# OpenDriveLab/kai0

Hardware: AMD Instinct MI355X
Metric: train samples/sec pi0.5 full FT (higher is better)
Workload: dtype bf16; 1 GPU; pi0.5 full fine-tune bf16, batch 32 per MI355X, 3-cam 224x224 (BASELINE.json configs[1]); global_batch=32, seq_len=1018, parallelism=dp1

## Files before the change

### include/kai0hip.h

```cpp
#ifndef KAI0HIP_H
#define KAI0HIP_H

#include <stdint.h>

#ifdef __cplusplus
extern "C" {
#endif

typedef void* kai0_stream_t;

const char* kai0_last_error(void);
int kai0_abi_version(void);
int kai0_device_info(int device, int* n_cu, int* lds_bytes, char* arch_name64);

typedef struct kai0_gemm_desc {
    const void* A;
    const void* B;
    void* C;
    int32_t M, N, K;
    int32_t a_kc, b_kc;
    int64_t lda, ldb, ldc;
    int32_t batch, batch_inner;
    int64_t sA1, sA2, sB1, sB2, sC1, sC2;
    int32_t a_rpb, b_rpb, c_rpb, _pad0;
// ... 126 lines not shown
int kai0_adarms_bwd(const void* dy, const void* dgate, const void* x, const float* mod, const float* rstd,
                    void* dx, float* dmod, const void* dres, int64_t rows, int rows_per_batch, int D,
                    kai0_stream_t stream);
int kai0_adarms_combine(const float* partials, int splits, int64_t split_stride, const void* gate_prev,
                        const void* residual, void* x_out, const float* mod, void* y, void* gate_out, int64_t rows,
                        int rows_per_batch, int D, float eps, kai0_stream_t stream);
int kai0_layernorm_fwd(const void* x, const void* w, const void* b, void* y, float* mean, float* rstd,
                       int64_t rows, int D, float eps, kai0_stream_t stream);
int kai0_layernorm_bwd(const void* dy, const void* x, const void* w, const float* mean, const float* rstd,
                       void* dx, float* dwb_partial, int dwb_blocks, const void* dres, int64_t rows, int D,
                       kai0_stream_t stream);
int kai0_reduce_partials(const float* partial, int blocks, int ncols, int64_t ld, void* out, int out_f32,
                         kai0_stream_t stream);
typedef struct kai0_reduce_item {
    const float* partial;
    void* out;
    int64_t ld;
    int32_t blocks, ncols;
    int32_t out_f32, _pad;
} kai0_reduce_item;
int kai0_reduce_partials_batch(const kai0_reduce_item* items, int n, kai0_stream_t stream);
int kai0_colsum_partials_bf16(const void* dy, int64_t M, int N, int64_t ld, float* scratch, int scratch_blocks,
                              int* blocks_used, kai0_stream_t stream);
int kai0_colsum_bf16(const void* dy, int64_t M, int N, int64_t ld, float* scratch, int scratch_blocks,
                     void* out, int out_f32, kai0_stream_t stream);

int kai0_rope_inplace(void* x, const int32_t* pos, const float* inv_freq, int B, int S, int64_t s_ld_rows,
                      int64_t row0, int H, int HD, int inverse, kai0_stream_t stream);
int kai0_rope_inplace2(void* x, int H, void* x2, int H2, const int32_t* pos, const float* inv_freq, int B, int S,
                       int64_t s_ld_rows, int64_t row0, int HD, kai0_stream_t stream);
int kai0_rope_copy(const void* src, void* dst, const int32_t* pos, const float* inv_freq, int B, int S, int H, int HD,
                   int64_t src_bs, int64_t src_ld, int64_t dst_bs, int64_t dst_ld, int64_t pos_bs, int inverse,
                   kai0_stream_t stream);

int kai0_softmax_mask_fwd(const void* scores, void* probs, const int32_t* qcode, const int32_t* kcode,
                          int B, int Sq, int H, int Sk, int64_t ld, int64_t batch_stride, int q0,
                          int64_t qcode_ld, int64_t kcode_ld, kai0_stream_t stream);
int kai0_siglip_attn_bwd(const void* q, const void* k, const void* v, const void* dO, const void* O, const void* P,
                         void* dq, void* dk, void* dv, int n_img, int S, int NH, int HD, int64_t ldp, int64_t ld_grad,
                         float scale, kai0_stream_t stream);
int kai0_siglip_attn_fwd(const void* q, const void* k, const void* v, void* o, float* lse, int n_img, int S, int NH, int HD,
                         int64_t ldq, int64_t ldk, int64_t ldv, int64_t ldo, int64_t sq, int64_t sk, int64_t sv, int64_t so,
                         float scale, kai0_stream_t stream);
int kai0_siglip_attn_bwd2(const void* q, const void* k, const void* v, const void* dO, const void* O, const float* lse,
                          void* dq, void* dk, void* dv, int n_img, int S, int NH, int HD, int64_t ld_grad, float scale,
                          kai0_stream_t stream);
int kai0_rowdot_bf16(const void* a, const void* b, float* out, int64_t rows, int D, kai0_stream_t stream);
int kai0_softmax_bwd(const void* probs, const void* dprobs, int dprobs_f32, void* dscores, int64_t rows, int Sk,
                     int64_t ld, float scale, kai0_stream_t stream);

typedef struct kai0_attn_desc {
    const void* Q; const void* K; const void* V; void* O; void* P;
    const int32_t* qcode; const int32_t* kcode;
    int32_t rows, Sk, HD, H, q0, batch, batch_inner, _pad0;
    int64_t ldq, ldk, ldv, ldo, ldp;
    int64_t sQ1, sQ2, sK1, sK2, sV1, sV2, sO1, sO2, sP;
    int64_t qcode_ld, kcode_ld;
    float scale;
    int32_t online;
    float* lse;
    int64_t s_lse;
} kai0_attn_desc;
int kai0_attn_fwd(const kai0_attn_desc* d, kai0_stream_t stream);
int kai0_attn_combine(const void* o_parts, const float* lse_parts, void* O, int parts, int rows, int HD, int64_t ldo,
                      int64_t part_stride, int64_t lse_stride, kai0_stream_t stream);
int kai0_attn_desc_size(void);

int kai0_geglu_fwd(const void* g, const void* u, void* h, int64_t n, kai0_stream_t stream);
int kai0_geglu_bwd(const void* dh, const void* g, const void* u, void* dg, void* du, int64_t n,
                   kai0_stream_t stream);
int kai0_gelu_bwd(const void* dy, const void* pre, void* dx, int64_t n, kai0_stream_t stream);
int kai0_silu_fwd_f32(const float* x, float* y, int64_t n, kai0_stream_t stream);
int kai0_silu_bwd_f32(const float* dy, const float* x, float* dx, int64_t n, kai0_stream_t stream);
int kai0_gated_fwd(const void* x, const void* y, const void* gate, void* out, int64_t rows, int rows_per_batch,
                   int D, kai0_stream_t stream);
int kai0_gated_bwd(const void* dout, const void* y, const void* gate, void* dy, void* dgate, int64_t rows,
                   int rows_per_batch, int D, kai0_stream_t stream);
int kai0_embed_gather(const void* table, const int64_t* tokens, void* out, int B, int T, int D, float scale,
                      int64_t out_bs, int64_t out_row0, int64_t out_ld, kai0_stream_t stream);
int kai0_embed_grad(const void* dout, const int64_t* tokens, void* dtable, int B, int T, int D, float scale,
                    int64_t dout_bs, int64_t dout_row0, int64_t dout_ld, kai0_stream_t stream);
int kai0_cast_f32_to_bf16(const float* x, void* y, int64_t n, kai0_stream_t stream);
int kai0_cast_bf16_to_f32(const void* x, float* y, int64_t n, kai0_stream_t stream);
int kai0_add_bf16(const void* a, const void* b, void* out, int64_t n, kai0_stream_t stream);
int kai0_add_f32(const float* a, const float* b, float* out, int64_t n, kai0_stream_t stream);
int kai0_transpose_bf16(const void* src, void* dst, int R, int C, kai0_stream_t stream);
typedef struct kai0_ck_item {
    const void* ptr;
    int64_t nbytes;
} kai0_ck_item;
int kai0_sampled_checksum(const kai0_ck_item* items_dev, int n, int stride, unsigned long long* out_dev, kai0_stream_t stream);
typedef struct kai0_pack_part {
    const void* src;
    void* dst;
    int64_t src_bs, src_ld, dst_bs, dst_ld;
    int32_t B, rows, cols, mode;
    int32_t pos_off, _pad;
} kai0_pack_part;
int kai0_pack_rows(const kai0_pack_part* parts, int n, const int32_t* pos, int64_t pos_bs, const float* inv_freq, int HD,
                   kai0_stream_t stream);
int kai0_copy_rows_bf16(const void* src, void* dst, int B, int rows, int D, int64_t src_bs, int64_t src_row0,
                        int64_t src_ld, int64_t dst_bs, int64_t dst_row0, int64_t dst_ld,
                        kai0_stream_t stream);
int kai0_patch_im2col(const float* img, float* cols, int n_img, int C, int HW, int P, kai0_stream_t stream);
int kai0_add_pos_cast(const float* x, const float* pos, void* out, int64_t rows, int n_pos, int D,
                      kai0_stream_t stream);

// ... 27 lines not shown
```

### kai0_amd/_lib.py

```python

from __future__ import annotations

import ctypes as C
import os
import pathlib

_HERE = pathlib.Path(__file__).resolve().parent
LIB_PATH = _HERE / "lib" / "libkai0hip.so"

c_p = C.c_void_p
c_i = C.c_int
c_i64 = C.c_int64
c_f = C.c_float


class GemmSeg(C.Structure):
    _fields_ = [("dst", c_p), ("ld", c_i64), ("n_begin", C.c_int32), ("_pad", C.c_int32)]


class GemmDesc(C.Structure):

    _fields_ = [
        ("A", c_p), ("B", c_p), ("C", c_p),
        ("M", C.c_int32), ("N", C.c_int32), ("K", C.c_int32),
        ("a_kc", C.c_int32), ("b_kc", C.c_int32),
        ("lda", c_i64), ("ldb", c_i64), ("ldc", c_i64),
        ("batch", C.c_int32), ("batch_inner", C.c_int32),
        ("sA1", c_i64), ("sA2", c_i64), ("sB1", c_i64), ("sB2", c_i64), ("sC1", c_i64), ("sC2", c_i64),
        ("a_rpb", C.c_int32), ("b_rpb", C.c_int32), ("c_rpb", C.c_int32), ("_pad0", C.c_int32),
        ("a_bs", c_i64), ("a_off", c_i64), ("b_bs", c_i64), ("b_off", c_i64), ("c_bs", c_i64), ("c_off", c_i64),
        ("bias", c_p), ("bias_f32", C.c_int32), ("scale", c_f),
        ("act", C.c_int32), ("out_f32", C.c_int32),
        ("pre_out", c_p), ("gate", c_p), ("gate_rpb", C.c_int32), ("accumulate", C.c_int32),
        ("gate_ld", c_i64), ("residual", c_p), ("ldr", c_i64), ("sR1", c_i64), ("sR2", c_i64),
        ("split_k", C.c_int32), ("c_nontemporal", C.c_int32), ("workspace", c_p), ("workspace_bytes", c_i64),
        ("aux1", c_p), ("aux2", c_p),
        ("nseg", C.c_int32), ("_pad2", C.c_int32), ("seg", GemmSeg * 3),
        ("rowvec", c_p), ("rv_s1", c_i64), ("rv_s2", c_i64), ("rv_ld", c_i64),
        ("B2", c_p), ("pre_out2", c_p),
        ("norm_out", c_p), ("norm_w", c_p), ("norm_b", c_p), ("norm_eps", C.c_float), ("norm_kind", C.c_int32),
        ("rope_cos", c_p), ("rope_sin", c_p), ("rope_half", C.c_int32), ("rope_n_end", C.c_int32),
        ("tile_cfg", C.c_int32), ("persist", C.c_int32), ("general_epilogue", C.c_int32), ("small_w8", C.c_int32),
    ]


class AttnDesc(C.Structure):

    _fields_ = [
        ("Q", c_p), ("K", c_p), ("V", c_p), ("O", c_p), ("P", c_p), ("qcode", c_p), ("kcode", c_p),
        ("rows", C.c_int32), ("Sk", C.c_int32), ("HD", C.c_int32), ("H", C.c_int32), ("q0", C.c_int32),
        ("batch", C.c_int32), ("batch_inner", C.c_int32), ("_pad0", C.c_int32),
        ("ldq", c_i64), ("ldk", c_i64), ("ldv", c_i64), ("ldo", c_i64), ("ldp", c_i64),
        ("sQ1", c_i64), ("sQ2", c_i64), ("sK1", c_i64), ("sK2", c_i64), ("sV1", c_i64), ("sV2", c_i64),
        ("sO1", c_i64), ("sO2", c_i64), ("sP", c_i64), ("qcode_ld", c_i64), ("kcode_ld", c_i64),
        ("scale", c_f), ("online", C.c_int32), ("lse", c_p), ("s_lse", c_i64),
    ]


class AttnBwdDesc(C.Structure):

    _fields_ = [
        ("dO", c_p), ("O", c_p), ("Q", c_p), ("K", c_p), ("V", c_p), ("lse", c_p), ("qcode", c_p), ("kcode", c_p),
        ("P", c_p), ("dS", c_p), ("dQ", c_p),
        ("batch", C.c_int32), ("rows", C.c_int32), ("Sk", C.c_int32), ("HD", C.c_int32), ("H", C.c_int32), ("_pad0", C.c_int32),
        ("ldo", c_i64), ("ldk", c_i64), ("ldv", c_i64), ("ldp", c_i64), ("sO", c_i64), ("sK", c_i64), ("sV", c_i64), ("sP", c_i64),
        ("s_lse", c_i64), ("qcode_ld", c_i64), ("kcode_ld", c_i64),
        ("scale", c_f), ("_pad1", C.c_int32),
    ]


class SkinnySeg(C.Structure):
    _fields_ = [("dst", c_p), ("ld", c_i64), ("n_begin", C.c_int32), ("n_end", C.c_int32), ("rope", C.c_int32),
                ("_pad", C.c_int32)]


class ReduceItem(C.Structure):

    _fields_ = [("partial", c_p), ("out", c_p), ("ld", c_i64), ("blocks", C.c_int32), ("ncols", C.c_int32),
                ("out_f32", C.c_int32), ("_pad", C.c_int32)]


class PackPart(C.Structure):

    _fields_ = [("src", c_p), ("dst", c_p), ("src_bs", c_i64), ("src_ld", c_i64), ("dst_bs", c_i64), ("dst_ld", c_i64),
                ("B", C.c_int32), ("rows", C.c_int32), ("cols", C.c_int32), ("mode", C.c_int32), ("pos_off", C.c_int32),
                ("_pad", C.c_int32)]


class SkinnyDesc(C.Structure):

    _fields_ = [
        ("A", c_p), ("W", c_p), ("lda", c_i64), ("ldw", c_i64),
        ("M", C.c_int32), ("N", C.c_int32), ("K", C.c_int32),
        ("pair_stride", C.c_int32), ("mode", C.c_int32), ("split_k", C.c_int32),
        ("a_rpb", C.c_int32), ("c_rpb", C.c_int32),
        ("a_bs", c_i64), ("a_off", c_i64), ("c_bs", c_i64), ("c_off", c_i64),
        ("seg", SkinnySeg * 3), ("nseg", C.c_int32), ("gate_rpb", C.c_int32),
        ("gate", c_p), ("gate_ld", c_i64), ("residual", c_p), ("ldr", c_i64),
        ("rope_cos", c_p), ("rope_sin", c_p), ("rope_half", C.c_int32), ("w_packed", C.c_int32),
        ("workspace", c_p), ("workspace_bytes", c_i64),
        ("mod", c_p), ("mod_ld", c_i64), ("mod_rpb", C.c_int32), ("eps", c_f),
        ("rowsq_in", c_p), ("cvec", c_p), ("rowsq_parts", C.c_int32), ("_pad2", C.c_int32), ("rowsq_ld", c_i64),
        ("rowsq_out", c_p), ("rowsq_out_ld", c_i64),
    ]
# ... 129 lines not shown
```

### kai0_amd/csrc/attention.hip

```cpp
#include "common.h"
#include "../../include/kai0hip.h"
#include <limits.h>
#include <stdlib.h>

namespace {

constexpr uint32_t OOB = 0x80000000u;
#ifdef KAI0_ABLATE
#define KAI0_ABL(p) ((p).ablate)
#else
#define KAI0_ABL(p) 0
#endif
constexpr int KC_LDS_MAX = 2048;

__device__ __forceinline__ void glds16(__amdgpu_buffer_rsrc_t rsrc, uint32_t voff, char* lds_dst_wave_uniform) {
    __builtin_amdgcn_raw_ptr_buffer_load_lds(rsrc, (LDS_PTR(void))lds_dst_wave_uniform, 16, (int)voff, 0, 0, 0);
}
__device__ __forceinline__ void lds_barrier() {
    __builtin_amdgcn_sched_barrier(0);
    asm volatile("s_waitcnt lgkmcnt(0)" ::: "memory");
    __builtin_amdgcn_s_barrier();
    asm volatile("" ::: "memory");
    __builtin_amdgcn_sched_barrier(0);
}

typedef __attribute__((ext_vector_type(4))) unsigned int u32x4;
typedef __attribute__((ext_vector_type(4))) int i32x4v;

struct AttnArgs {
    const bf16_t* Q;
    const bf16_t* K;
    const bf16_t* V;
    bf16_t* O;
    bf16_t* P;
    const int32_t* qcode;
    const int32_t* kcode;
    int rows, Sk, HD, H, q0;
    int64_t ldq, ldk, ldv, ldo, ldp;
    int batch_inner;
    int64_t sQ1, sQ2, sK1, sK2, sV1, sV2, sO1, sO2, sP;
    int64_t qcode_ld, kcode_ld;
    float scale;
    int kc_lds_keys;
    float* lse;
    int64_t s_lse;
    int nt_p;
    int ablate;
};

template <int NKS, int VC, int QT, int OP = 0, int RB = 128>
__global__ __launch_bounds__(RB / (16 * QT) * 64, RB == 64 ? 2 : 1) void attn_fwd_kernel(const AttnArgs p) {
    constexpr int WAVES = RB / (16 * QT);
    constexpr int NST = RB == 64 ? 1 : 2;
    static_assert(RB == 128 && QT == 1, "128-row blocks of eight waves (the 64-row / four-wave forms were measured slower and removed)");
    constexpr int OMT = VC / 16;
    constexpr int KSTEPS = NKS * 2;
    constexpr int K_BYTES = NKS * 8192;
    constexpr int V_ROWB = VC * 2;
    constexpr int V_BYTES = 64 * V_ROWB;
    constexpr int STAGE = K_BYTES + V_BYTES;
    constexpr int V_LPR = V_ROWB / 16;
    constexpr int V_RPP = 64 / V_LPR;
    constexpr int NKP = NKS * 8 / WAVES;
    constexpr int NVP = (64 / V_RPP) / WAVES;
    static_assert(NKP >= 1 && NVP >= 1, "too many waves for this tile");
    extern __shared__ __attribute__((aligned(16))) char smem[];
    char* pbuf_all = smem + (OP > 0 ? OP : NST) * STAGE;
    int* kc_lds = reinterpret_cast<int*>(pbuf_all + WAVES * QT * 2048);

    const int tid = threadIdx.x, lane = tid & 63;
    const int wave = __builtin_amdgcn_readfirstlane(tid >> 6);
    const int l15 = lane & 15, g = lane >> 4;
    const int z = blockIdx.y;
    const int z1 = z / p.batch_inner, z2 = z - z1 * p.batch_inner;
    const bf16_t* Qb = p.Q + z1 * p.sQ1 + z2 * p.sQ2;
    const bf16_t* Kb = p.K + z1 * p.sK1 + z2 * p.sK2;
    const bf16_t* Vb = p.V + z1 * p.sV1 + z2 * p.sV2;
    bf16_t* Ob = p.O + z1 * p.sO1 + z2 * p.sO2;
    bf16_t* Pb = p.P + (int64_t)z * p.sP;
    const __amdgpu_buffer_rsrc_t k_rsrc = __builtin_amdgcn_make_buffer_rsrc((void*)Kb, 0, (int)OOB, 0x00020000);
    const __amdgpu_buffer_rsrc_t v_rsrc = __builtin_amdgcn_make_buffer_rsrc((void*)Vb, 0, (int)OOB, 0x00020000);
    const __amdgpu_buffer_rsrc_t p_rsrc = __builtin_amdgcn_make_buffer_rsrc((void*)Pb, 0, (int)OOB, 0x00020000);
    const int row0 = blockIdx.x * RB + wave * (16 * QT);
    const int ntiles = (p.Sk + 63) / 64;
    const uint32_t ldk2 = (uint32_t)p.ldk * 2, ldv2 = (uint32_t)p.ldv * 2;

    const __amdgpu_buffer_rsrc_t q_rsrc = __builtin_amdgcn_make_buffer_rsrc((void*)Qb, 0, (int)OOB, 0x00020000);
    bf16x8 qf[QT][KSTEPS];
#pragma unroll
    for (int nt = 0; nt < QT; ++nt) {
        const int r = row0 + nt * 16 + l15;
#pragma unroll
        for (int ks = 0; ks < KSTEPS; ++ks) {
            const int d = ks * 32 + g * 8;
            const uint32_t off = (r < p.rows && d < p.HD) ? (uint32_t)r * (uint32_t)(p.ldq * 2) + (uint32_t)d * 2 : OOB;
            qf[nt][ks] = __builtin_bit_cast(bf16x8, __builtin_amdgcn_raw_buffer_load_b128(q_rsrc, (int)off, 0, 0));
        }
    }
    int qc[QT];
#pragma unroll
    for (int nt = 0; nt < QT; ++nt) {
        const int r = row0 + nt * 16 + l15;
        qc[nt] = INT_MAX;
        if (p.qcode != nullptr) qc[nt] = r < p.rows ? p.qcode[z1 * p.qcode_ld + p.q0 + r / p.H] : -1;
    }

    const int kc_chunk = ((lane & 7) ^ (lane >> 3)) * 8;
    auto stage = [&](int kt, int slot, bool with_v) {
        char* sk = smem + slot * STAGE + wave * (NKP * 1024);
        char* sv = smem + slot * STAGE + K_BYTES + wave * (NVP * 1024);
        const int key0 = kt * 64;
#pragma unroll
        for (int j = 0; j < NKP; ++j) {
            const int piece = wave * NKP + j;
            const int sub = piece >> 3, key = key0 + (piece & 7) * 8 + (lane >> 3);
            const int d = sub * 64 + kc_chunk;
            const uint32_t off = (key < p.Sk && d < p.HD) ? (uint32_t)key * ldk2 + (uint32_t)d * 2 : OOB;
            glds16(k_rsrc, off, sk + j * 1024);
        }
        if (with_v) {
#pragma unroll
            for (int j = 0; j < NVP; ++j) {
                const int r = (wave * NVP + j) * V_RPP + lane / V_LPR;
                const int c = (lane % V_LPR) ^ ((r & 7) << 1);
                const int key = key0 + r;
                const uint32_t off = (key < p.Sk && c * 8 < p.HD) ? (uint32_t)key * ldv2 + (uint32_t)c * 16 : OOB;
                glds16(v_rsrc, off, sv + j * 1024);
            }
        }
    };

    auto logits_f = [&](const char* tk, f32x4 (&s)[4][QT], auto&& fill) {
#pragma unroll
        for (int mt = 0; mt < 4; ++mt)
#pragma unroll
            for (int nt = 0; nt < QT; ++nt) s[mt][nt] = f32x4{0.f, 0.f, 0.f, 0.f};
        bf16x8 kf[2][4];
        auto rd = [&](int ks, bf16x8 (&dst)[4]) {
            const char* sub = tk + (ks >> 1) * 8192;
            const int chunk = (ks & 1) * 4 + g;
#pragma unroll
            for (int mt = 0; mt < 4; ++mt) {
                const int row = mt * 16 + l15;
                dst[mt] = *reinterpret_cast<const bf16x8*>(sub + row * 128 + ((chunk ^ (row & 7)) << 4));
            }
        };
        rd(0, kf[0]);
#pragma unroll
        for (int ks = 0; ks < KSTEPS; ++ks) {
            if (ks + 1 < KSTEPS) rd(ks + 1, kf[(ks + 1) & 1]);
            __builtin_amdgcn_sched_barrier(0);
#pragma unroll
            for (int mt = 0; mt < 4; ++mt)
#pragma unroll
                for (int nt = 0; nt < QT; ++nt)
                    s[mt][nt] = __builtin_amdgcn_mfma_f32_16x16x32_bf16(kf[ks & 1][mt], qf[nt][ks], s[mt][nt], 0, 0, 0);
            fill(ks);
            __builtin_amdgcn_sched_barrier(0);
        }
    };
    auto logits = [&](const char* tk, f32x4 (&s)[4][QT]) { logits_f(tk, s, [](int) {}); };
    if (p.kc_lds_keys > 0) {
        for (int i = tid; i < p.kc_lds_keys; i += WAVES * 64)
            kc_lds[i] = p.kcode == nullptr ? 0 : (i < p.Sk ? p.kcode[z1 * p.kcode_ld + i] : INT_MAX);
    }
    auto load_kcodes = [&](int kt, int (&kc)[4][4]) {
        if (p.kc_lds_keys > 0) {
#pragma unroll
            for (int mt = 0; mt < 4; ++mt) {
                const i32x4v c = *reinterpret_cast<const i32x4v*>(kc_lds + kt * 64 + mt * 16 + 4 * g);
#pragma unroll
                for (int r = 0; r < 4; ++r) kc[mt][r] = c[r];
            }
            return;
        }
#pragma unroll
        for (int mt = 0; mt < 4; ++mt) {
            const int key = kt * 64 + mt * 16 + 4 * g;
#pragma unroll
            for (int r = 0; r < 4; ++r)
                kc[mt][r] = p.kcode == nullptr ? 0 : ((key + r < p.Sk) ? p.kcode[z1 * p.kcode_ld + key + r] : INT_MAX);
        }
// ... 122 lines not shown
#pragma unroll
                for (int mt = 0; mt < 4; ++mt)
#pragma unroll
                    for (int r = 0; r < 4; ++r) m_run[nt] = fmaxf(m_run[nt], sall[t][mt][nt][r]);
        }
#pragma unroll
        for (int nt = 0; nt < QT; ++nt) {
            float m = m_run[nt];
            m = fmaxf(m, __shfl_xor(m, 16, 64));
            m = fmaxf(m, __shfl_xor(m, 32, 64));
            float l = 0.f;
            if (m > -INFINITY) {
#pragma unroll
                for (int t = 0; t < OP; ++t)
#pragma unroll
                    for (int mt = 0; mt < 4; ++mt)
#pragma unroll
                        for (int r = 0; r < 4; ++r) l += __expf(sall[t][mt][nt][r] - m);
            }
            l += __shfl_xor(l, 16, 64);
            l += __shfl_xor(l, 32, 64);
            m_run[nt] = m;
            inv_l[nt] = l > 0.f ? 1.0f / l : 0.f;
            const int r = row0 + nt * 16 + l15;
            if (p.lse != nullptr && g == 0 && r < p.rows) p.lse[(int64_t)z * p.s_lse + r] = l > 0.f ? m + __logf(l) : INFINITY;
        }
#pragma unroll
        for (int t = 0; t < OP; ++t)
            if (t < ntiles) emit_tile(t, smem + t * STAGE + K_BYTES, sall[t], m_run, inv_l);
    } else if constexpr (OP < 0) {
        float m_run[QT], l_run[QT];
#pragma unroll
        for (int nt = 0; nt < QT; ++nt) { m_run[nt] = -INFINITY; l_run[nt] = 0.f; }
        int* lt = kc_lds + KC_LDS_MAX;
        const bool use_list = p.kc_lds_keys > 0;
        int nlive = ntiles;
        if (use_list) {
            __syncthreads();
            for (int t = wave; t < ntiles; t += WAVES) {
                const bool any = __any(kc_lds[t * 64 + lane] != INT_MAX);
                if (lane == 0) lt[40 + t] = any ? 1 : 0;
            }
            __syncthreads();
            if (tid == 0) {
                int n = 0;
                for (int t = 0; t < ntiles; ++t)
                    if (lt[40 + t]) lt[1 + n++] = t;
                lt[0] = n;
            }
            __syncthreads();
            nlive = __builtin_amdgcn_readfirstlane(lt[0]);
        }
        auto tile_at = [&](int i) -> int { return use_list ? __builtin_amdgcn_readfirstlane(lt[1 + i]) : i; };
        if (nlive > 0) stage(tile_at(0), 0, true);
        asm volatile("s_waitcnt vmcnt(0)" ::: "memory");
        lds_barrier();
        for (int it = 0; it < nlive; ++it) {
            const int kt = tile_at(it);
            const int buf = NST == 2 ? (it & 1) : 0;
            if (NST == 2 && it + 1 < nlive && !(KAI0_ABL(p) & 8)) stage(tile_at(it + 1), buf ^ 1, true);
            const char* tk = smem + buf * STAGE;
            int kc[4][4];
            load_kcodes(kt, kc);
            f32x4 s[4][QT];
            if (KAI0_ABL(p) & 16) {
#pragma unroll
                for (int mt = 0; mt < 4; ++mt)
#pragma unroll
                    for (int nt = 0; nt < QT; ++nt) s[mt][nt] = f32x4{0.f, 0.f, 0.f, 0.f};
            } else
            logits(tk, s);
            finish_logits(kt, s, kc);
            bf16x4 pb[4][QT];
#pragma unroll
            for (int nt = 0; nt < QT; ++nt) {
                float tmax = -INFINITY;
#pragma unroll
                for (int mt = 0; mt < 4; ++mt)
#pragma unroll
                    for (int r = 0; r < 4; ++r) tmax = fmaxf(tmax, s[mt][nt][r]);
                tmax = fmaxf(tmax, __shfl_xor(tmax, 16, 64));
                tmax = fmaxf(tmax, __shfl_xor(tmax, 32, 64));
                const float mn = fmaxf(m_run[nt], tmax);
                const bool live = mn > -INFINITY;
                const float alpha = live ? __expf(m_run[nt] - mn) : 1.0f;
                float lsum = 0.f;
#pragma unroll
                for (int mt = 0; mt < 4; ++mt)
#pragma unroll
                    for (int r = 0; r < 4; ++r) {
                        const float e = (KAI0_ABL(p) & 32) ? s[mt][nt][r] : live ? __expf(s[mt][nt][r] - mn) : 0.f;
                        lsum += e;
                        pb[mt][nt][r] = f2bf(e);
                    }
                l_run[nt] = l_run[nt] * alpha + lsum;
                m_run[nt] = mn;
                if (__any(alpha != 1.0f)) {
#pragma unroll
                    for (int mt = 0; mt < OMT; ++mt) o[mt][nt] *= alpha;
                }
            }
            pv_tile(tk + K_BYTES, pb);
            if (NST == 1) {
                lds_barrier();
                if (it + 1 < nlive) stage(tile_at(it + 1), 0, true);
            }
            asm volatile("s_waitcnt vmcnt(0)" ::: "memory");
            lds_barrier();
        }
#pragma unroll
        for (int nt = 0; nt < QT; ++nt) {
            float l = l_run[nt];
            l += __shfl_xor(l, 16, 64);
            l += __shfl_xor(l, 32, 64);
            const float inv = l > 0.f ? 1.0f / l : 0.f;
#pragma unroll
            for (int mt = 0; mt < OMT; ++mt) o[mt][nt] *= inv;
            const int r = row0 + nt * 16 + l15;
            if (p.lse != nullptr && g == 0 && r < p.rows) p.lse[(int64_t)z * p.s_lse + r] = l > 0.f ? m_run[nt] + __logf(l) : INFINITY;
        }
    } else {
    float m_run[QT], l_run[QT];
#pragma unroll
    for (int nt = 0; nt < QT; ++nt) { m_run[nt] = -INFINITY; l_run[nt] = 0.f; }
    stage(0, 0, false);
    asm volatile("s_waitcnt vmcnt(0)" ::: "memory");
    lds_barrier();
    for (int kt = 0; kt < ((KAI0_ABL(p) & 2) ? 0 : ntiles); ++kt) {
        const int buf = NST == 2 ? (kt & 1) : 0;
        if (NST == 2 && kt + 1 < ntiles && !(KAI0_ABL(p) & 8)) stage(kt + 1, buf ^ 1, false);
        int kc[4][4];
        load_kcodes(kt, kc);
        f32x4 s[4][QT];
        logits(smem + buf * STAGE, s);
        finish_logits(kt, s, kc);
#pragma unroll
        for (int nt = 0; nt < QT; ++nt) {
            float tmax = -INFINITY;
#pragma unroll
            for (int mt = 0; mt < 4; ++mt)
#pragma unroll
                for (int r = 0; r < 4; ++r) tmax = fmaxf(tmax, s[mt][nt][r]);
            const float mn = fmaxf(m_run[nt], tmax);
            if (mn > -INFINITY) {
                float acc = l_run[nt] * __expf(m_run[nt] - mn);
#pragma unroll
                for (int mt = 0; mt < 4; ++mt)
#pragma unroll
                    for (int r = 0; r < 4; ++r) acc += __expf(s[mt][nt][r] - mn);
                l_run[nt] = acc;
                m_run[nt] = mn;
            }
        }
        if (NST == 1) {
            lds_barrier();
            if (kt + 1 < ntiles && !(KAI0_ABL(p) & 8)) stage(kt + 1, 0, false);
        }
        asm volatile("s_waitcnt vmcnt(0)" ::: "memory");
        lds_barrier();
    }
    float inv_l[QT];
// ... 87 lines not shown
        }
    }
    const float inv = wsum > 0.f ? 1.0f / wsum : 0.f;
    bf16x8 o;
#pragma unroll
    for (int e = 0; e < 8; ++e) o[e] = f2bf(acc[e] * inv);
    *reinterpret_cast<bf16x8*>(O + (int64_t)r * ldo + c) = o;
}

}

KAI0_API int kai0_attn_combine(const void* o_parts, const float* lse_parts, void* O, int parts, int rows, int HD, int64_t ldo,
                               int64_t part_stride, int64_t lse_stride, kai0_stream_t stream) {
    KAI0_REQUIRE(o_parts && lse_parts && O, "kai0_attn_combine: null operand");
    KAI0_REQUIRE(parts >= 1 && parts <= 8 && HD % 8 == 0 && HD > 0 && ldo % 8 == 0 && part_stride % 8 == 0 && lse_stride >= rows &&
                     ((uintptr_t)o_parts % 16) == 0 && ((uintptr_t)O % 16) == 0,
                 "kai0_attn_combine: 1..8 parts, HD %% 8 == 0, 16-byte aligned rows");
    if (rows <= 0) return 0;
    const int64_t n = (int64_t)rows * (HD / 8);
    hipLaunchKernelGGL(attn_combine_kernel, dim3((unsigned)((n + 255) / 256)), dim3(256), 0, (hipStream_t)stream, (const bf16_t*)o_parts,
                       lse_parts, (bf16_t*)O, parts, rows, HD, ldo, part_stride, lse_stride);
    return kai0_check_launch("kai0_attn_combine");
}

KAI0_API int kai0_attn_desc_size(void) { return (int)sizeof(kai0_attn_desc); }

KAI0_API int kai0_attn_fwd(const kai0_attn_desc* d, kai0_stream_t stream) {
    KAI0_REQUIRE(d != nullptr && d->Q && d->K && d->V && d->O, "kai0_attn_fwd: null operand");
    KAI0_REQUIRE(d->HD % 8 == 0 && d->HD > 0 && d->HD <= 256, "kai0_attn_fwd: HD=%d unsupported", d->HD);
    KAI0_REQUIRE(d->ldq % 8 == 0 && d->ldk % 8 == 0 && d->ldv % 8 == 0 && d->ldo % 4 == 0,
                 "kai0_attn_fwd: leading dims must be multiples of 8");
    KAI0_REQUIRE(d->P == nullptr || (d->ldp % 8 == 0 && d->ldp >= d->Sk && d->ldp <= ((d->Sk + 63) / 64) * 64),
                 "kai0_attn_fwd: ldp=%lld must be a multiple of 8 in [Sk, round_up(Sk, 64)]", (long long)d->ldp);
    KAI0_REQUIRE((d->qcode == nullptr) == (d->kcode == nullptr), "kai0_attn_fwd: qcode/kcode must both be set");
    KAI0_REQUIRE(d->H >= 1, "kai0_attn_fwd: H must be >= 1");
    KAI0_REQUIRE((int64_t)d->Sk * d->ldk * 2 < (int64_t)0x7FFF0000 && (int64_t)d->Sk * d->ldv * 2 < (int64_t)0x7FFF0000,
                 "kai0_attn_fwd: K/V span more than 2 GiB per batch entry");
    KAI0_REQUIRE(d->P == nullptr || (int64_t)d->rows * d->ldp * 2 < (int64_t)0x7FFF0000, "kai0_attn_fwd: P spans more than 2 GiB per batch entry");
    KAI0_REQUIRE((int64_t)d->rows * d->ldq * 2 < (int64_t)0x7FFF0000, "kai0_attn_fwd: Q spans more than 2 GiB per batch entry");
    if (d->rows <= 0 || d->Sk <= 0) return 0;
    AttnArgs p;
    p.Q = (const bf16_t*)d->Q; p.K = (const bf16_t*)d->K; p.V = (const bf16_t*)d->V;
    p.O = (bf16_t*)d->O; p.P = (bf16_t*)d->P;
    p.qcode = d->qcode; p.kcode = d->kcode;
    p.rows = d->rows; p.Sk = d->Sk; p.HD = d->HD; p.H = d->H; p.q0 = d->q0;
    p.ldq = d->ldq; p.ldk = d->ldk; p.ldv = d->ldv; p.ldo = d->ldo; p.ldp = d->ldp;
    p.batch_inner = d->batch_inner > 0 ? d->batch_inner : 1;
    p.sQ1 = d->sQ1; p.sQ2 = d->sQ2; p.sK1 = d->sK1; p.sK2 = d->sK2; p.sV1 = d->sV1; p.sV2 = d->sV2;
    p.sO1 = d->sO1; p.sO2 = d->sO2; p.sP = d->sP;
    p.qcode_ld = d->qcode_ld; p.kcode_ld = d->kcode_ld;
    p.scale = d->scale;
    p.lse = d->lse; p.s_lse = d->s_lse;
    KAI0_REQUIRE(d->lse == nullptr || d->s_lse >= d->rows, "kai0_attn_fwd: s_lse=%lld < rows", (long long)d->s_lse);
#ifdef KAI0_ABLATE
    static const int ablate = [] { const char* e = getenv("KAI0_ATTN_ABLATE"); return e ? atoi(e) : 0; }();
    p.ablate = ablate;
#else
    p.ablate = 0;
#endif
    p.nt_p = 1;
    const int kc_keys = ((d->Sk + 63) / 64) * 64;
    p.kc_lds_keys = kc_keys <= KC_LDS_MAX ? kc_keys : 0;
    const int batch = d->batch > 0 ? d->batch : 1;
    dim3 grid((d->rows + 127) / 128, batch, 1);
    hipStream_t s = (hipStream_t)stream;
#define KAI0_ATTN_LAUNCH(NKS, VC, QT, OP, RB)                                                                          \
    do {                                                                                                          \
        constexpr int LDS = (OP > 0 ? OP : (RB == 64 ? 1 : 2)) * (NKS * 8192 + 64 * VC * 2) + (RB / 32) * 4096 + KC_LDS_MAX * 4 + 512; \
        static_assert(LDS <= 160 * 1024, "attention LDS budget");                                                    \
        static bool attr_set = false;                                                                             \
        auto kern = attn_fwd_kernel<NKS, VC, QT, OP, RB>;                                                             \
        if (!attr_set) {                                                                                          \
            hipError_t e = hipFuncSetAttribute((const void*)kern, hipFuncAttributeMaxDynamicSharedMemorySize, LDS); \
            KAI0_REQUIRE(e == hipSuccess, "kai0_attn_fwd: cannot reserve %d B of LDS: %s", LDS, hipGetErrorString(e)); \
            attr_set = true;                                                                                      \
        }                                                                                                         \
        hipLaunchKernelGGL(kern, grid, dim3(RB / (16 * QT) * 64), LDS, s, p);                                    \
    } while (0)
    KAI0_REQUIRE(d->online != 1 || d->P == nullptr, "kai0_attn_fwd: the one-pass form does not produce P");
    const bool online = d->P == nullptr && d->online != 2;
    if (d->HD <= 128) {
        if (d->Sk <= 256 && (int64_t)grid.x * grid.y <= 512) KAI0_ATTN_LAUNCH(2, 128, 1, 4, 128);
        else if (online) KAI0_ATTN_LAUNCH(2, 128, 1, -1, 128);
        else KAI0_ATTN_LAUNCH(2, 128, 1, 0, 128);
    } else {
        if (online) KAI0_ATTN_LAUNCH(4, 256, 1, -1, 128);
        else KAI0_ATTN_LAUNCH(4, 256, 1, 0, 128);
    }
#undef KAI0_ATTN_LAUNCH
    return kai0_check_launch("kai0_attn_fwd");
}
```

### kai0_amd/ops.py

```python

from __future__ import annotations

import contextlib
import ctypes as C
import os
import math

import torch

from . import _lib
from ._lib import AttnBwdDesc, AttnDesc, GemmDesc

BF16 = torch.bfloat16
F32 = torch.float32

NORM_PARTIAL_BLOCKS = 512
COLSUM_BLOCKS = 256


def _stream() -> int:
    return torch.cuda.current_stream().cuda_stream


def _p(t: torch.Tensor | None) -> int | None:
# ... 1132 lines not shown
        ones = torch.ones((1, rows), dtype=F32, device=dout.device)
        gemm_f32(ones, rows, 1, d32, D, 1, db.view(1, D), 1, D, rows)
        GG = G * G
        dpos = _grad_dst(ppos, F32)
        if n == 1:
            dpos.copy_(d32)
        else:
            ones_n = torch.ones((1, n), dtype=F32, device=dout.device)
            gemm_f32(ones_n, n, 1, d32.view(n, GG * D), GG * D, 1, dpos.view(1, GG * D), 1, GG * D, n)
        return None, _grad_ret(pw, dw.view(wshape)), _grad_ret(pb, db), _grad_ret(ppos, dpos), None


def patch_embed(img, w, b, pos, patch):
    return PatchEmbedFn.apply(img, w, b, pos, patch)


def _copy_rows(src, dst, Bn, rows, D, sbs, sr0, sld, dbs, dr0, dld):
    _lib.call("kai0_copy_rows_bf16", src.data_ptr(), dst.data_ptr(), Bn, rows, D, sbs, sr0, sld, dbs, dr0, dld, _stream())


def rope_(x, pos, inv_freq, Bn, S, s_ld, row0, H, HD, inverse=False):
    _lib.call("kai0_rope_inplace", x.data_ptr(), pos.data_ptr(), inv_freq.data_ptr(), Bn, S, s_ld, row0, H, HD,
              int(inverse), _stream())


def rope2_(x, H, x2, H2, pos, inv_freq, Bn, S, s_ld, row0, HD):
    _lib.call("kai0_rope_inplace2", x.data_ptr(), H, x2.data_ptr(), H2, pos.data_ptr(), inv_freq.data_ptr(), Bn, S, s_ld, row0, HD,
              _stream())


def rope_copy(src_t, dst_t, pos, inv_freq, Bn, S, H, HD, *, src, dst, pos_bs, pos_off=0, inverse=False):
    sbs, sld, sr0 = src
    dbs, dld, dr0 = dst
    _lib.call("kai0_rope_copy", src_t.data_ptr() + 2 * sr0 * sld, dst_t.data_ptr() + 2 * dr0 * dld, pos.data_ptr() + 4 * pos_off,
              inv_freq.data_ptr(), Bn, S, H, HD, sbs, sld, dbs, dld, pos_bs, int(inverse), _stream())


def pack_rows(parts, HD: int, pos=None, pos_bs: int = 0, inv_freq=None):
    for c0 in range(0, len(parts), 12):
        chunk = parts[c0 : c0 + 12]
        arr = (_lib.PackPart * len(chunk))()
        for a, (src, soff, dst, doff, (sbs, sld), (dbs, dld), Bn, rows, cols, mode, pos_off) in zip(arr, chunk):
            a.src = None if src is None else src.data_ptr() + 2 * soff
            a.dst = dst.data_ptr() + 2 * doff
            a.src_bs, a.src_ld, a.dst_bs, a.dst_ld = sbs, sld, dbs, dld
            a.B, a.rows, a.cols, a.mode, a.pos_off = Bn, rows, cols, mode, pos_off
        _lib.call("kai0_pack_rows", C.addressof(arr), len(chunk), _p(pos), pos_bs, _p(inv_freq), HD, _stream())


def round_up(x: int, m: int) -> int:
    return (x + m - 1) // m * m


def attn_fwd_keysplit(Q, K, V, O, *, rows, Sk, HD, H, q0, ldk, ldv, qcode, kcode, scale, q_off, o_off, parts: int = 4):
    if Sk % parts != 0:
        raise ValueError("attn_fwd_keysplit: Sk must be a multiple of the number of key ranges")
    rng = Sk // parts
    dev = Q.device
    o_parts = torch.empty((parts, rows, HD), dtype=BF16, device=dev)
    lse = torch.empty((parts, rows), dtype=torch.float32, device=dev)
    d = AttnDesc()
    d.Q, d.K, d.V, d.O = Q.data_ptr() + 2 * q_off, K.data_ptr(), V.data_ptr(), o_parts.data_ptr()
    d.qcode, d.kcode = _p(qcode), _p(kcode)
    d.rows, d.Sk, d.HD, d.H, d.q0, d.batch, d.batch_inner = rows, rng, HD, H, q0, parts, 1
    d.ldq, d.ldk, d.ldv, d.ldo = HD, ldk, ldv, HD
    d.sQ1, d.sK1, d.sV1, d.sO1 = 0, rng * ldk, rng * ldv, rows * HD
    d.qcode_ld, d.kcode_ld = 0, rng
    d.scale = scale
    d.online = 1
    d.lse, d.s_lse = lse.data_ptr(), rows
    _lib.call("kai0_attn_fwd", C.byref(d), _stream())
    _lib.call("kai0_attn_combine", o_parts.data_ptr(), lse.data_ptr(), O.data_ptr() + 2 * o_off, parts, rows, HD, HD, rows * HD, rows, _stream())


def attn_fwd(Q, K, V, O, P, *, rows, Sk, HD, H=1, q0=0, batch=1, batch_inner=1, ldq, ldk, ldv, ldo, ldp=0, sQ=(0, 0),
             sK=(0, 0), sV=(0, 0), sO=(0, 0), sP=0, qcode=None, kcode=None, scale, q_off=0, o_off=0, lse=None, online=0):
    d = AttnDesc()
    d.Q, d.K, d.V, d.O = Q.data_ptr() + 2 * q_off, K.data_ptr(), V.data_ptr(), O.data_ptr() + 2 * o_off
    d.P = _p(P)
    d.qcode, d.kcode = _p(qcode), _p(kcode)
    d.rows, d.Sk, d.HD, d.H, d.q0, d.batch, d.batch_inner = rows, Sk, HD, H, q0, batch, batch_inner
    d.ldq, d.ldk, d.ldv, d.ldo, d.ldp = ldq, ldk, ldv, ldo, ldp
    d.sQ1, d.sQ2 = sQ
    d.sK1, d.sK2 = sK
    d.sV1, d.sV2 = sV
    d.sO1, d.sO2 = sO
    d.sP = sP
    if qcode is not None:
        d.qcode_ld, d.kcode_ld = qcode.stride(0), kcode.stride(0)
    d.scale = scale
    d.online = online
    if lse is not None:
        _chk(lse, torch.float32, "lse")
        d.lse, d.s_lse = lse.data_ptr(), lse.stride(0)
    _lib.call("kai0_attn_fwd", C.byref(d), _stream())


_ATTN_STORE_P = os.environ.get("KAI0_ATTN_STORE_P", "0") == "1"


def mqa_attention_fwd(q_all, k_all, v_all, qcode, kcode, Bn, Sq, q0, Sk, S_ld, H, HD, scale, want_probs=True, want_lse=False):
    dev = q_all.device
    M = Sq * H
    if want_lse:
        lse = torch.empty((Bn, M), dtype=torch.float32, device=dev)
        att = torch.empty((Bn, S_ld, H * HD), dtype=BF16, device=dev)
        attn_fwd(q_all, k_all, v_all, att, None, rows=M, Sk=Sk, HD=HD, H=H, q0=q0, batch=Bn, ldq=HD, ldk=HD, ldv=HD, ldo=HD,
                 sQ=(S_ld * H * HD, 0), sK=(S_ld * HD, 0), sV=(S_ld * HD, 0), sO=(S_ld * H * HD, 0), qcode=qcode, kcode=kcode,
                 scale=scale, q_off=q0 * H * HD, o_off=q0 * H * HD, lse=lse)
        return att, lse
    probs = torch.empty((Bn, M, S_ld), dtype=BF16, device=dev) if want_probs else None
    att = torch.empty((Bn, S_ld, H * HD), dtype=BF16, device=dev)
    attn_fwd(q_all, k_all, v_all, att, probs, rows=M, Sk=Sk, HD=HD, H=H, q0=q0, batch=Bn, ldq=HD, ldk=HD, ldv=HD, ldo=HD,
             ldp=S_ld, sQ=(S_ld * H * HD, 0), sK=(S_ld * HD, 0), sV=(S_ld * HD, 0), sO=(S_ld * H * HD, 0), sP=M * S_ld,
             qcode=qcode, kcode=kcode, scale=scale, q_off=q0 * H * HD, o_off=q0 * H * HD)
    return att, probs


def _attn_bwd_split(Bn: int, S_ld: int, HD: int, M: int) -> int:
    t256 = ((S_ld + 255) // 256) * ((HD + 255) // 256) * Bn
    if t256 >= 160 or M < 4096:
        return 1
    return max(1, min(8, -(-256 // t256), M // 2048))


def _joint_attention_grads(cfg, pos, inv_freq, dq_all, dk_all, dv_all):
    Bn, S, S_ld, H, HD, seg_lens, scale, recompute = cfg
    dev = dq_all.device
    grads, parts = [], []
    r0 = 0
    for Li in seg_lens:
        W3 = (H + 2) * HD
        dq, dk, dv = fused_columns(Bn * Li, (H * HD, HD, HD), dev)
        parts.append((dq_all, r0 * H * HD, dq, 0, (S_ld * H * HD, H * HD), (Li * W3, W3), Bn, Li, H * HD, 2, r0))
        parts.append((dk_all, r0 * HD, dk, 0, (dk_all.stride(0), HD), (Li * W3, W3), Bn, Li, HD, 2, r0))
        parts.append((dv_all, r0 * HD, dv, 0, (dv_all.stride(0), HD), (Li * W3, W3), Bn, Li, HD, 0, 0))
        grads += [dq, dk, dv]
        r0 += Li
    pack_rows(parts, HD, pos, S, inv_freq)
    return (None, None, None, None, None, None, None, *grads)


class JointAttentionFn(torch.autograd.Function):

# ... 225 lines not shown
```

Baseline: 69.01 samples/s.

## Add ping-pong two-group schedule to one-pass attention forward kernel

Adds a ping-pong variant of the online attention forward kernel. Two groups of four waves alternate between issuing K/V loads and doing matmul or softmax work, and s_setprio raises priority for the MFMA phases. The goal is to overlap global-to-LDS staging and softmax with the QK and PV matrix work instead of running them in lockstep. It becomes the default (sched=0) for the online path, which adds more barriers and a more complex double-buffer protocol, with a risk of races or extra synchronization cost.

```diff
diff --git a/include/kai0hip.h b/include/kai0hip.h
--- a/include/kai0hip.h
+++ b/include/kai0hip.h
@@ -202,7 +202,8 @@
 typedef struct kai0_attn_desc {
     const void* Q; const void* K; const void* V; void* O; void* P;
     const int32_t* qcode; const int32_t* kcode;
-    int32_t rows, Sk, HD, H, q0, batch, batch_inner, _pad0;
+    int32_t rows, Sk, HD, H, q0, batch, batch_inner;
+    int32_t sched;
     int64_t ldq, ldk, ldv, ldo, ldp;
     int64_t sQ1, sQ2, sK1, sK2, sV1, sV2, sO1, sO2, sP;
     int64_t qcode_ld, kcode_ld;
diff --git a/kai0_amd/_lib.py b/kai0_amd/_lib.py
--- a/kai0_amd/_lib.py
+++ b/kai0_amd/_lib.py
@@ -49,7 +49,7 @@
     _fields_ = [
         ("Q", c_p), ("K", c_p), ("V", c_p), ("O", c_p), ("P", c_p), ("qcode", c_p), ("kcode", c_p),
         ("rows", C.c_int32), ("Sk", C.c_int32), ("HD", C.c_int32), ("H", C.c_int32), ("q0", C.c_int32),
-        ("batch", C.c_int32), ("batch_inner", C.c_int32), ("_pad0", C.c_int32),
+        ("batch", C.c_int32), ("batch_inner", C.c_int32), ("sched", C.c_int32),
         ("ldq", c_i64), ("ldk", c_i64), ("ldv", c_i64), ("ldo", c_i64), ("ldp", c_i64),
         ("sQ1", c_i64), ("sQ2", c_i64), ("sK1", c_i64), ("sK2", c_i64), ("sV1", c_i64), ("sV2", c_i64),
         ("sO1", c_i64), ("sO2", c_i64), ("sP", c_i64), ("qcode_ld", c_i64), ("kcode_ld", c_i64),
diff --git a/kai0_amd/csrc/attention.hip b/kai0_amd/csrc/attention.hip
--- a/kai0_amd/csrc/attention.hip
+++ b/kai0_amd/csrc/attention.hip
@@ -45,10 +45,11 @@
     float* lse;
     int64_t s_lse;
     int nt_p;
+    int sched;
     int ablate;
 };
 
-template <int NKS, int VC, int QT, int OP = 0, int RB = 128>
+template <int NKS, int VC, int QT, int OP = 0, int RB = 128, bool PP = false>
 __global__ __launch_bounds__(RB / (16 * QT) * 64, RB == 64 ? 2 : 1) void attn_fwd_kernel(const AttnArgs p) {
     constexpr int WAVES = RB / (16 * QT);
     constexpr int NST = RB == 64 ? 1 : 2;
@@ -64,6 +65,7 @@
     constexpr int NKP = NKS * 8 / WAVES;
     constexpr int NVP = (64 / V_RPP) / WAVES;
     static_assert(NKP >= 1 && NVP >= 1, "too many waves for this tile");
+    static_assert(!PP || (OP < 0 && WAVES == 8), "ping-pong: the one-pass form on eight waves");
     extern __shared__ __attribute__((aligned(16))) char smem[];
     char* pbuf_all = smem + (OP > 0 ? OP : NST) * STAGE;
     int* kc_lds = reinterpret_cast<int*>(pbuf_all + WAVES * QT * 2048);
@@ -106,9 +108,8 @@
     }
 
     const int kc_chunk = ((lane & 7) ^ (lane >> 3)) * 8;
-    auto stage = [&](int kt, int slot, bool with_v) {
+    auto stage_k = [&](int kt, int slot) {
         char* sk = smem + slot * STAGE + wave * (NKP * 1024);
-        char* sv = smem + slot * STAGE + K_BYTES + wave * (NVP * 1024);
         const int key0 = kt * 64;
 #pragma unroll
         for (int j = 0; j < NKP; ++j) {
@@ -118,16 +119,22 @@
             const uint32_t off = (key < p.Sk && d < p.HD) ? (uint32_t)key * ldk2 + (uint32_t)d * 2 : OOB;
             glds16(k_rsrc, off, sk + j * 1024);
         }
-        if (with_v) {
-#pragma unroll
-            for (int j = 0; j < NVP; ++j) {
-                const int r = (wave * NVP + j) * V_RPP + lane / V_LPR;
-                const int c = (lane % V_LPR) ^ ((r & 7) << 1);
-                const int key = key0 + r;
-                const uint32_t off = (key < p.Sk && c * 8 < p.HD) ? (uint32_t)key * ldv2 + (uint32_t)c * 16 : OOB;
-                glds16(v_rsrc, off, sv + j * 1024);
-            }
-        }
+    };
+    auto stage_v = [&](int kt, int slot) {
+        char* sv = smem + slot * STAGE + K_BYTES + wave * (NVP * 1024);
+        const int key0 = kt * 64;
+#pragma unroll
+        for (int j = 0; j < NVP; ++j) {
+            const int r = (wave * NVP + j) * V_RPP + lane / V_LPR;
+            const int c = (lane % V_LPR) ^ ((r & 7) << 1);
+            const int key = key0 + r;
+            const uint32_t off = (key < p.Sk && c * 8 < p.HD) ? (uint32_t)key * ldv2 + (uint32_t)c * 16 : OOB;
+            glds16(v_rsrc, off, sv + j * 1024);
+        }
+    };
+    auto stage = [&](int kt, int slot, bool with_v) {
+        stage_k(kt, slot);
+        if (with_v) stage_v(kt, slot);
     };
 
     auto logits_f = [&](const char* tk, f32x4 (&s)[4][QT], auto&& fill) {
@@ -356,6 +363,78 @@
             nlive = __builtin_amdgcn_readfirstlane(lt[0]);
         }
         auto tile_at = [&](int i) -> int { return use_list ? __builtin_amdgcn_readfirstlane(lt[1 + i]) : i; };
+        auto softmax_tile = [&](f32x4 (&s)[4][QT], bf16x4 (&pb)[4][QT]) {
+#pragma unroll
+            for (int nt = 0; nt < QT; ++nt) {
+                float tmax = -INFINITY;
+#pragma unroll
+                for (int mt = 0; mt < 4; ++mt)
+#pragma unroll
+                    for (int r = 0; r < 4; ++r) tmax = fmaxf(tmax, s[mt][nt][r]);
+                tmax = fmaxf(tmax, __shfl_xor(tmax, 16, 64));
+                tmax = fmaxf(tmax, __shfl_xor(tmax, 32, 64));
+                const float mn = fmaxf(m_run[nt], tmax);
+                const bool live = mn > -INFINITY;
+                const float alpha = live ? __expf(m_run[nt] - mn) : 1.0f;
+                float lsum = 0.f;
+#pragma unroll
+                for (int mt = 0; mt < 4; ++mt)
+#pragma unroll
+                    for (int r = 0; r < 4; ++r) {
+                        const float e = (KAI0_ABL(p) & 32) ? s[mt][nt][r] : live ? __expf(s[mt][nt][r] - mn) : 0.f;
+                        lsum += e;
+                        pb[mt][nt][r] = f2bf(e);
+                    }
+                l_run[nt] = l_run[nt] * alpha + lsum;
+                m_run[nt] = mn;
+                if (__any(alpha != 1.0f)) {
+#pragma unroll
+                    for (int mt = 0; mt < OMT; ++mt) o[mt][nt] *= alpha;
+                }
+            }
+        };
+        if constexpr (PP) {
+            const int grp = wave >> 2;
+            bf16x4 pb[4][QT];
+            f32x4 s[4][QT];
+            int kc[4][4];
+            int kt = 0;
+            if (nlive > 0) stage_k(tile_at(0), 0);
+            asm volatile("s_waitcnt vmcnt(0)" ::: "memory");
+            lds_barrier();
+            if (grp == 1) {
+                if (1 < nlive) stage_k(tile_at(1), 1);
+                if (0 < nlive) stage_v(tile_at(0), 0);
+                lds_barrier();
+            }
+            for (int j = 0; j <= nlive; ++j) {
+                if (grp == 0) {
+                    if (j + 1 < nlive) stage_k(tile_at(j + 1), (j + 1) & 1);
+                    if (j < nlive) stage_v(tile_at(j), j & 1);
+                }
+                if (j < nlive) {
+                    kt = tile_at(j);
+                    load_kcodes(kt, kc);
+                }
+                __builtin_amdgcn_s_setprio(1);
+                if (j > 0) pv_tile(smem + ((j - 1) & 1) * STAGE + K_BYTES, pb);
+                if (j < nlive) logits(smem + (j & 1) * STAGE, s);
+                __builtin_amdgcn_s_setprio(0);
+                if (grp == 1) asm volatile("s_waitcnt vmcnt(0)" ::: "memory");
+                lds_barrier();
+                if (grp == 1) {
+                    if (j + 2 < nlive) stage_k(tile_at(j + 2), j & 1);
+                    if (j + 1 < nlive) stage_v(tile_at(j + 1), (j + 1) & 1);
+                }
+                if (j < nlive) {
+                    finish_logits(kt, s, kc);
+                    softmax_tile(s, pb);
+                }
+                if (grp == 0) asm volatile("s_waitcnt vmcnt(0)" ::: "memory");
+                lds_barrier();
+            }
+            if (grp == 0) lds_barrier();
+        } else {
         if (nlive > 0) stage(tile_at(0), 0, true);
         asm volatile("s_waitcnt vmcnt(0)" ::: "memory");
         lds_barrier();
@@ -376,34 +455,7 @@
             logits(tk, s);
             finish_logits(kt, s, kc);
             bf16x4 pb[4][QT];
-#pragma unroll
-            for (int nt = 0; nt < QT; ++nt) {
-                float tmax = -INFINITY;
-#pragma unroll
-                for (int mt = 0; mt < 4; ++mt)
-#pragma unroll
-                    for (int r = 0; r < 4; ++r) tmax = fmaxf(tmax, s[mt][nt][r]);
-                tmax = fmaxf(tmax, __shfl_xor(tmax, 16, 64));
-                tmax = fmaxf(tmax, __shfl_xor(tmax, 32, 64));
-                const float mn = fmaxf(m_run[nt], tmax);
-                const bool live = mn > -INFINITY;
-                const float alpha = live ? __expf(m_run[nt] - mn) : 1.0f;
-                float lsum = 0.f;
-#pragma unroll
-                for (int mt = 0; mt < 4; ++mt)
-#pragma unroll
-                    for (int r = 0; r < 4; ++r) {
-                        const float e = (KAI0_ABL(p) & 32) ? s[mt][nt][r] : live ? __expf(s[mt][nt][r] - mn) : 0.f;
-                        lsum += e;
-                        pb[mt][nt][r] = f2bf(e);
-                    }
-                l_run[nt] = l_run[nt] * alpha + lsum;
-                m_run[nt] = mn;
-                if (__any(alpha != 1.0f)) {
-#pragma unroll
-                    for (int mt = 0; mt < OMT; ++mt) o[mt][nt] *= alpha;
-                }
-            }
+            softmax_tile(s, pb);
             pv_tile(tk + K_BYTES, pb);
             if (NST == 1) {
                 lds_barrier();
@@ -411,6 +463,7 @@
             }
             asm volatile("s_waitcnt vmcnt(0)" ::: "memory");
             lds_barrier();
+        }
         }
 #pragma unroll
         for (int nt = 0; nt < QT; ++nt) {
@@ -604,6 +657,7 @@
     p.scale = d->scale;
     p.lse = d->lse; p.s_lse = d->s_lse;
     KAI0_REQUIRE(d->lse == nullptr || d->s_lse >= d->rows, "kai0_attn_fwd: s_lse=%lld < rows", (long long)d->s_lse);
+    KAI0_REQUIRE(d->sched == 0 || d->sched == 1, "kai0_attn_fwd: sched=%d must be 0 (ping-pong) or 1 (one phase)", d->sched);
 #ifdef KAI0_ABLATE
     static const int ablate = [] { const char* e = getenv("KAI0_ATTN_ABLATE"); return e ? atoi(e) : 0; }();
     p.ablate = ablate;
@@ -611,17 +665,18 @@
     p.ablate = 0;
 #endif
     p.nt_p = 1;
+    p.sched = d->sched;
     const int kc_keys = ((d->Sk + 63) / 64) * 64;
     p.kc_lds_keys = kc_keys <= KC_LDS_MAX ? kc_keys : 0;
     const int batch = d->batch > 0 ? d->batch : 1;
     dim3 grid((d->rows + 127) / 128, batch, 1);
     hipStream_t s = (hipStream_t)stream;
-#define KAI0_ATTN_LAUNCH(NKS, VC, QT, OP, RB)                                                                          \
+#define KAI0_ATTN_LAUNCH(NKS, VC, QT, OP, RB, ...)                                                                     \
     do {                                                                                                          \
         constexpr int LDS = (OP > 0 ? OP : (RB == 64 ? 1 : 2)) * (NKS * 8192 + 64 * VC * 2) + (RB / 32) * 4096 + KC_LDS_MAX * 4 + 512; \
         static_assert(LDS <= 160 * 1024, "attention LDS budget");                                                    \
         static bool attr_set = false;                                                                             \
-        auto kern = attn_fwd_kernel<NKS, VC, QT, OP, RB>;                                                             \
+        auto kern = attn_fwd_kernel<NKS, VC, QT, OP, RB, ##__VA_ARGS__>;                                              \
         if (!attr_set) {                                                                                          \
             hipError_t e = hipFuncSetAttribute((const void*)kern, hipFuncAttributeMaxDynamicSharedMemorySize, LDS); \
             KAI0_REQUIRE(e == hipSuccess, "kai0_attn_fwd: cannot reserve %d B of LDS: %s", LDS, hipGetErrorString(e)); \
@@ -631,12 +686,15 @@
     } while (0)
     KAI0_REQUIRE(d->online != 1 || d->P == nullptr, "kai0_attn_fwd: the one-pass form does not produce P");
     const bool online = d->P == nullptr && d->online != 2;
+    const bool pp = d->sched == 0;
     if (d->HD <= 128) {
         if (d->Sk <= 256 && (int64_t)grid.x * grid.y <= 512) KAI0_ATTN_LAUNCH(2, 128, 1, 4, 128);
+        else if (online && pp) KAI0_ATTN_LAUNCH(2, 128, 1, -1, 128, true);
         else if (online) KAI0_ATTN_LAUNCH(2, 128, 1, -1, 128);
         else KAI0_ATTN_LAUNCH(2, 128, 1, 0, 128);
     } else {
-        if (online) KAI0_ATTN_LAUNCH(4, 256, 1, -1, 128);
+        if (online && pp) KAI0_ATTN_LAUNCH(4, 256, 1, -1, 128, true);
+        else if (online) KAI0_ATTN_LAUNCH(4, 256, 1, -1, 128);
         else KAI0_ATTN_LAUNCH(4, 256, 1, 0, 128);
     }
 #undef KAI0_ATTN_LAUNCH
diff --git a/kai0_amd/ops.py b/kai0_amd/ops.py
--- a/kai0_amd/ops.py
+++ b/kai0_amd/ops.py
@@ -1208,7 +1208,7 @@
     return (x + m - 1) // m * m
 
 
-def attn_fwd_keysplit(Q, K, V, O, *, rows, Sk, HD, H, q0, ldk, ldv, qcode, kcode, scale, q_off, o_off, parts: int = 4):
+def attn_fwd_keysplit(Q, K, V, O, *, rows, Sk, HD, H, q0, ldk, ldv, qcode, kcode, scale, q_off, o_off, parts: int = 4, sched: int = 0):
     if Sk % parts != 0:
         raise ValueError("attn_fwd_keysplit: Sk must be a multiple of the number of key ranges")
     rng = Sk // parts
@@ -1224,13 +1224,14 @@
     d.qcode_ld, d.kcode_ld = 0, rng
     d.scale = scale
     d.online = 1
+    d.sched = sched
     d.lse, d.s_lse = lse.data_ptr(), rows
     _lib.call("kai0_attn_fwd", C.byref(d), _stream())
     _lib.call("kai0_attn_combine", o_parts.data_ptr(), lse.data_ptr(), O.data_ptr() + 2 * o_off, parts, rows, HD, HD, rows * HD, rows, _stream())
 
 
 def attn_fwd(Q, K, V, O, P, *, rows, Sk, HD, H=1, q0=0, batch=1, batch_inner=1, ldq, ldk, ldv, ldo, ldp=0, sQ=(0, 0),
-             sK=(0, 0), sV=(0, 0), sO=(0, 0), sP=0, qcode=None, kcode=None, scale, q_off=0, o_off=0, lse=None, online=0):
+             sK=(0, 0), sV=(0, 0), sO=(0, 0), sP=0, qcode=None, kcode=None, scale, q_off=0, o_off=0, lse=None, online=0, sched=0):
     d = AttnDesc()
     d.Q, d.K, d.V, d.O = Q.data_ptr() + 2 * q_off, K.data_ptr(), V.data_ptr(), O.data_ptr() + 2 * o_off
     d.P = _p(P)
@@ -1246,6 +1247,7 @@
         d.qcode_ld, d.kcode_ld = qcode.stride(0), kcode.stride(0)
     d.scale = scale
     d.online = online
+    d.sched = sched
     if lse is not None:
         _chk(lse, torch.float32, "lse")
         d.lse, d.s_lse = lse.data_ptr(), lse.stride(0)
```

After: 68.54 samples/s (median of 3 runs). Within noise of the previous version (-0.7%).
